# ppwwyyxx/OpenPano

Hardware: NVIDIA H100
Metric: Mpixels/sec SIFT+match+blend (higher is better)
Workload: dtype f32

## Files before the change

openpano_b200/csrc/blur_tile.cuh:

```cuda
#pragma once
#include "common.cuh"

#define BT_W 64
#define BT_H 32
#define BT_THREADS 256

struct BlurTile { int om; int tx, ty; };

__device__ __forceinline__ BlurTile find_blur_tile(const int2* __restrict__ span, int n_om, int cta) {
  int lo = 0, hi = n_om - 1;
  while (lo < hi) {
    const int mid = (lo + hi + 1) >> 1;
    if (span[mid].x <= cta) lo = mid; else hi = mid - 1;
  }
  const int local = cta - span[lo].x, tx_n = span[lo].y;
  BlurTile t;
  t.om = lo; t.ty = local / tx_n; t.tx = local - t.ty * tx_n;
  return t;
}

__device__ __forceinline__ float2 fmul2(float2 a, float t) { return make_float2(__fmul_rn(a.x, t), __fmul_rn(a.y, t)); }

#define BLUR_COLBUF_FLOATS(C) (16 * ((((BT_W + 2 * (C) + 2) / 2) * 2) | 1) * 2)

template <int C>
__device__ __forceinline__ void blur_level(const float* __restrict__ grey, float* __restrict__ colbuf,
                                           float* __restrict__ outT, const float* __restrict__ taps_g,
                                           int R, int RX, int GW, int tid) {
  constexpr int KW = 2 * C + 1;
  float tap[KW];
#pragma unroll
  for (int k = 0; k < KW; ++k) tap[k] = taps_g[k];
  const int start = (RX - C) & ~1, off = (RX - C) - start;
  const int npair = (BT_W + 2 * C + off + 1) >> 1;
  const int csp = (2 * npair) | 1;
  float2* colbuf2 = reinterpret_cast<float2*>(colbuf);
  for (int item = tid; item < (BT_H / 8) * npair; item += BT_THREADS) {
    const int strip = item / npair, pr = item - strip * npair;
    const float2* col = reinterpret_cast<const float2*>(grey + (strip * 8 + R - C) * GW + start) + pr;
    const int gw2 = GW >> 1;
    float2 win[8 + 2 * C];
#pragma unroll
    for (int j = 0; j < 8 + 2 * C; ++j) win[j] = col[j * gw2];
#pragma unroll
    for (int r = 0; r < 8; r += 2) {
      float a0x = 0.f, a0y = 0.f, a1x = 0.f, a1y = 0.f;
#pragma unroll
      for (int k = 0; k < KW; ++k) {
        const float2 p0 = fmul2(win[r + k], tap[k]);
        const float2 p1 = fmul2(win[r + 1 + k], tap[k]);
        a0x += p0.x; a0y += p0.y; a1x += p1.x; a1y += p1.y;
      }
      float2* dst = colbuf2 + (strip * 4 + (r >> 1)) * csp + 2 * pr;
      dst[0] = make_float2(a0x, a1x);
      dst[1] = make_float2(a0y, a1y);
    }
  }
  __syncthreads();
  if (tid < 128) {
    const int lane = tid & 31, p = lane & 15, xs = ((tid >> 5) * 2 + (lane >> 4)) * 8;
    const float2* row = colbuf2 + p * csp + off + xs;
    float2 win[8 + 2 * C];
#pragma unroll
    for (int j = 0; j < 8 + 2 * C; ++j) win[j] = row[j];
#pragma unroll
    for (int c = 0; c < 8; ++c) {
      float ax = 0.f, ay = 0.f;
#pragma unroll
      for (int k = 0; k < KW; ++k) {
        const float2 pp = fmul2(win[c + k], tap[k]);
        ax += pp.x; ay += pp.y;
      }
      outT[(2 * p) * (BT_W + 1) + xs + c] = ax;
      outT[(2 * p + 1) * (BT_W + 1) + xs + c] = ay;
    }
  }
  __syncthreads();
}

__device__ __forceinline__ uint32_t sm_u32(const void* p) { return (uint32_t)__cvta_generic_to_shared(p); }
__device__ __forceinline__ void sbar_init(uint32_t bar, uint32_t count) {
  asm volatile("mbarrier.init.shared::cta.b64 [%0], %1;" ::"r"(bar), "r"(count));
}
__device__ __forceinline__ void sbar_expect_tx(uint32_t bar, uint32_t bytes) {
  asm volatile("mbarrier.arrive.expect_tx.shared::cta.b64 _, [%0], %1;" ::"r"(bar), "r"(bytes) : "memory");
}
__device__ __forceinline__ void sbar_wait(uint32_t bar, uint32_t parity) {
  uint32_t done = 0;
  for (uint32_t spin = 0; spin < (1u << 28); ++spin) {
    asm volatile(
        "{\n\t.reg .pred P1;\n\t"
        "mbarrier.try_wait.parity.shared::cta.b64 P1, [%1], %2;\n\t"
        "selp.b32 %0, 1, 0, P1;\n\t}"
        : "=r"(done) : "r"(bar), "r"(parity) : "memory");
    if (done) return;
  }
  __trap();
}
__device__ __forceinline__ void tma_load_2d(uint32_t dst, const TmaDesc* map, int cx, int cy, uint32_t bar) {
  asm volatile("fence.proxy.tensormap::generic.acquire.gpu [%0], 128;" ::"l"(map) : "memory");
  asm volatile(
      "cp.async.bulk.tensor.2d.shared::cluster.global.tile.mbarrier::complete_tx::bytes [%0], [%1, {%2, %3}], [%4];"
      ::"r"(dst), "l"(map), "r"(cx), "r"(cy), "r"(bar) : "memory");
}
```

openpano_b200/csrc/sift.cu:

```cuda
#include "sift.cuh"
#include "desc_interval.h"
#include <math.h>
#include <string.h>
#include <algorithm>
#include <map>
#include <mutex>
#include <cuda.h>

__device__ __forceinline__ void bilinear_coef(int d, float inv, int src_n, int* s, float* frac) {
  float r = ((float)d + 0.5f) * inv - 0.5f;
  int si = (int)floorf(r);
  r -= (float)si;
  if (si < 0) { si = 0; r = 0.f; }
  else if (si + 1 >= src_n) { si = src_n - 2; r = 1.f; }
  *s = si; *frac = r;
}

__device__ __forceinline__ int first_tap_at_least(int t, float inv, int src_n, int dst_n) {
  auto tap = [&](int d) { int s; float f; bilinear_coef(d, inv, src_n, &s, &f); return s; };
  int d = (int)fminf(fmaxf(((float)t + 0.5f) / inv - 0.5f, 0.f), (float)dst_n);
  while (d > 0 && tap(d - 1) >= t) --d;
  while (d < dst_n && tap(d) < t) ++d;
  return d;
}
// ... 52 lines not shown
    if (lc <= last_c) {
      int sy; float ry;
      bilinear_coef(C0 + lc, im.ify, im.in_w, &sy, &ry);
      for (int lr = threadIdx.x / PG_TW; lr <= last_r; lr += PG_ROWS_PER_PASS) stage(lr, lc, sy, ry);
    }
    const int hr = (int)threadIdx.x - (PG_THREADS - PG_TW);
    if (hr >= 0 && hr <= last_r && PG_TW <= last_c) {
      int sy; float ry;
      bilinear_coef(C0 + PG_TW, im.ify, im.in_w, &sy, &ry);
      stage(hr, PG_TW, sy, ry);
    }
  }
  if (n_oct == 1) return;
  __syncthreads();
  for (int o = 1; o < n_oct; ++o) {
    const OctMeta& om = octs[blockIdx.z * n_oct + o];
    const float ifx = om.ifx, ify = om.ify;
    const int d_r0 = first_tap_at_least(R0, ifx, im.h0, om.h), d_r1 = first_tap_at_least(R0 + PG_TH, ifx, im.h0, om.h);
    const int d_c0 = first_tap_at_least(C0, ify, im.w0, om.w), d_c1 = first_tap_at_least(C0 + PG_TW, ify, im.w0, om.w);
    const int nc = d_c1 - d_c0;
    if (nc == 0) continue;
    float* g = arena + om.gauss_off;
    const int pitch = om.pitch;
    const int step_r = PG_THREADS / nc, step_c = PG_THREADS - step_r * nc;
    int dr = d_r0 + (int)threadIdx.x / nc, dc = d_c0 + (int)threadIdx.x % nc;
    for (; dr < d_r1; dr += step_r, dc += step_c) {
      if (dc >= d_c1) { dc -= nc; ++dr; if (dr >= d_r1) break; }
      int sx, sy; float rx, ry;
      bilinear_coef(dr, ifx, im.h0, &sx, &rx);
      bilinear_coef(dc, ify, im.w0, &sy, &ry);
      const float irx = 1.0f - rx, iry = 1.0f - ry;
      const float* p0 = tile + (sx - R0) * SW + (sy - C0);
      const float* p1 = p0 + SW;
      float v[3];
#pragma unroll
      for (int ch = 0; ch < 3; ++ch)
        v[ch] = rx * (p1[ch * SP + 1] * ry + p1[ch * SP] * iry) + irx * (p0[ch * SP + 1] * ry + p0[ch * SP] * iry);
      g[(size_t)dr * pitch + dc] = (v[0] + v[1] + v[2]) / 3.f;
    }
  }
}

struct ExtremaParams {
  int nscale;
  float pre_color_thres, diff_thres;
  int cap;
  int* cand_count;
  uint32_t* cand_keys;
  int seam_cap;
  int* seam_count;
  uint32_t* seam_keys;
};

__device__ __forceinline__ uint32_t make_key(int oct, int scale, int y, int x) {
  return ((uint32_t)oct << 29) | ((uint32_t)scale << 26) | ((uint32_t)y << 13) | (uint32_t)x;
}

template <class DoG>
__device__ __forceinline__ bool is_extremum(float center, float pre_color_thres, float diff_thres, const DoG& dog) {
  if (center < pre_color_thres) return false;
  const float cmp1 = center - diff_thres, cmp2 = center + diff_thres;
  bool mx = true, mn = true;
#pragma unroll
  for (int ds = -1; ds <= 1; ++ds) {
#pragma unroll
    for (int di = -1; di <= 1; ++di)
#pragma unroll
      for (int dj = -1; dj <= 1; ++dj) {
        if (ds == 0 && di == 0 && dj == 0) continue;
        const float v = dog(ds, di, dj);
        if (v >= cmp1) mx = false;
        if (v <= cmp2) mn = false;
      }
    if (!mx && !mn) return false;
  }
  return true;
}

__device__ __forceinline__ void append_candidate(const ExtremaParams& ep, int img, uint32_t key) {
  const int slot = atomicAdd(&ep.cand_count[img], 1);
  if (slot < ep.cap) ep.cand_keys[(size_t)img * ep.cap + slot] = key;
}

#include "blur_tile.cuh"

__global__ void __launch_bounds__(BT_THREADS)
k_blur_dog(const OctMeta* __restrict__ octs, const int2* __restrict__ span, int n_om,
           float* __restrict__ arena, const __grid_constant__ GaussTable gt) {
  extern __shared__ float smem[];
  const BlurTile tl = find_blur_tile(span, n_om, blockIdx.x);
  const OctMeta om = octs[tl.om];
  const int R = gt.rmax;
  const int GW = BT_W + 2 * R;
  const int GH = BT_H + 2 * R;
  float* grey = smem;
  float* colbuf = smem + GH * GW;
  const int x0 = tl.tx * BT_W, y0 = tl.ty * BT_H;
  const float* g0 = arena + om.gauss_off;
  const int tid = threadIdx.x;

  for (int i = tid; i < GH * GW; i += BT_THREADS) {
    int yy = i / GW, xx = i - yy * GW;
    int gy = min(max(y0 + yy - R, 0), om.h - 1);
    int gx = min(max(x0 + xx - R, 0), om.w - 1);
    grey[i] = __ldg(g0 + (size_t)gy * om.pitch + gx);
  }
  __syncthreads();

  const int tx = tid & (BT_W - 1), ty = tid / BT_W;
  for (int s = 0; s < gt.nlev; ++s) {
    const int c = gt.center[s];
    const float* taps = gt.taps[s];
    const int cw = BT_W + 2 * c;
    for (int i = tid; i < BT_H * cw; i += BT_THREADS) {
      int y = i / cw, xx = i - y * cw;
      const float* col = grey + (y + R - c) * GW + (xx + R - c);
      float tmp = 0.f;
      for (int k = 0; k <= 2 * c; ++k) tmp += col[k * GW] * taps[k];
      colbuf[y * GW + xx] = tmp;
    }
    __syncthreads();
    float* lvl = arena + om.gauss_off + (size_t)(s + 1) * om.plane;
#pragma unroll
    for (int i = 0; i < BT_H / 4; ++i) {
      int y = ty + 4 * i;
      const float* row = colbuf + y * GW + tx;
      float tmp = 0.f;
      for (int k = 0; k <= 2 * c; ++k) tmp += row[k] * taps[k];
      int gx = x0 + tx, gy = y0 + y;
      if (gx < om.w && gy < om.h) lvl[(size_t)gy * om.pitch + gx] = tmp;
    }
    __syncthreads();
  }
}

#define EX_RING_FLOATS (3 * BT_H * BT_W)
__global__ void __launch_bounds__(BT_THREADS, 3)
k_blur_extrema(const OctMeta* __restrict__ octs, const int2* __restrict__ span, int n_om, int n_tiles,
               const TmaDesc* __restrict__ maps, float* __restrict__ arena, const __grid_constant__ GaussTable gt,
               const ExtremaParams ep) {
  extern __shared__ __align__(128) float smem[];
  __shared__ __align__(8) uint64_t s_bar[2];
  __shared__ BlurTile s_tile[2];
  const int R = gt.rmax;
  const int RX = (R + 3) & ~3;
  const int GW = BT_W + 2 * RX, GH = BT_H + 2 * R;
  const int GSZ = (GH * GW + 31) & ~31;
  float* grey0 = smem;
  float* colbuf = smem + 2 * GSZ;
  float* outT = colbuf + BLUR_COLBUF_FLOATS(6);
  float* ring = outT + BT_H * (BT_W + 1);
  const int tid = threadIdx.x;
  const uint32_t tile_bytes = (uint32_t)(GH * GW * sizeof(float));
  int t = blockIdx.x;
  if (tid == 0) {
    sbar_init(sm_u32(&s_bar[0]), 1);
    sbar_init(sm_u32(&s_bar[1]), 1);
    asm volatile("fence.mbarrier_init.release.cluster;" ::: "memory");
    if (t < n_tiles) {
      const BlurTile tl = find_blur_tile(span, n_om, t);
      s_tile[0] = tl;
      sbar_expect_tx(sm_u32(&s_bar[0]), tile_bytes);
      tma_load_2d(sm_u32(grey0), maps + tl.om, tl.tx * BT_W - RX, tl.ty * BT_H - R, sm_u32(&s_bar[0]));
    }
  }
  __syncthreads();
  for (int it = 0; t < n_tiles; t += gridDim.x, ++it) {
    const int b = it & 1;
    float* grey = grey0 + b * GSZ;
    const BlurTile tl = s_tile[b];
    const OctMeta om = octs[tl.om];
    const int x0 = tl.tx * BT_W, y0 = tl.ty * BT_H;
    if (tid == 0 && t + (int)gridDim.x < n_tiles) {
      const BlurTile nx = find_blur_tile(span, n_om, t + gridDim.x);
      s_tile[b ^ 1] = nx;
      asm volatile("fence.proxy.async.shared::cta;" ::: "memory");
      sbar_expect_tx(sm_u32(&s_bar[b ^ 1]), tile_bytes);
      tma_load_2d(sm_u32(grey0 + (b ^ 1) * GSZ), maps + nx.om, nx.tx * BT_W - RX, nx.ty * BT_H - R, sm_u32(&s_bar[b ^ 1]));
    }
    sbar_wait(sm_u32(&s_bar[b]), (uint32_t)(it >> 1) & 1u);
    if (x0 - RX < 0 || y0 - R < 0 || x0 + BT_W + RX > om.w || y0 + BT_H + R > om.h) {
      for (int i = tid; i < GH * GW; i += BT_THREADS) {
        const int yy = i / GW, xx = i - yy * GW;
        const int gy = y0 + yy - R, gx = x0 + xx - RX;
        const int cy = min(max(gy, 0), om.h - 1), cx = min(max(gx, 0), om.w - 1);
        if (cy != gy || cx != gx) grey[i] = grey[(cy - y0 + R) * GW + (cx - x0 + RX)];
      }
      __syncthreads();
    }
    const int tx = tid & (BT_W - 1), ty = tid / BT_W;
    const int gx = x0 + tx;
    const bool col_in = gx >= 1 && gx <= om.w - 2;
    const bool col_seam = tx == 0 || tx == BT_W - 1;
    float prev[BT_H / 4];
#pragma unroll
    for (int i = 0; i < BT_H / 4; ++i) prev[i] = grey[(ty + 4 * i + R) * GW + tx + RX];
    for (int s = 0; s < gt.nlev; ++s) {
      if (gt.center[s] == 3) blur_level<3>(grey, colbuf, outT, gt.taps[s], R, RX, GW, tid);
      else blur_level<6>(grey, colbuf, outT, gt.taps[s], R, RX, GW, tid);
      float* lvl = arena + om.gauss_off + (size_t)(s + 1) * om.plane;
      float* dog = ring + (s % 3) * (BT_H * BT_W);
#pragma unroll
      for (int i = 0; i < BT_H / 4; ++i) {
        const int y = ty + 4 * i, gy = y0 + y;
        const float v = outT[y * (BT_W + 1) + tx];
        if (gx < om.w && gy < om.h) lvl[(size_t)gy * om.pitch + gx] = v;
        dog[y * BT_W + tx] = fabsf(prev[i] - v);
        prev[i] = v;
      }
      if (s >= 2) {
        __syncthreads();
        const int j = s - 1;
        const float* d0 = ring + ((s - 2) % 3) * (BT_H * BT_W);
        const float* d1 = ring + ((s - 1) % 3) * (BT_H * BT_W);
        const float* d2 = dog;
#pragma unroll 1
        for (int i = 0; i < BT_H / 4; ++i) {
          const int y = ty + 4 * i, gy = y0 + y;
          if (!col_in || gy < 1 || gy > om.h - 2) continue;
          const int o = y * BT_W + tx;
          const float center = d1[o];
          if (center < ep.pre_color_thres) continue;
          if (col_seam || y == 0 || y == BT_H - 1) {
            const int slot = atomicAdd(&ep.seam_count[om.img], 1);
            if (slot < ep.seam_cap) ep.seam_keys[(size_t)om.img * ep.seam_cap + slot] = make_key(om.oct, j, gy, gx);
            continue;
          }
          auto at = [&](int ds, int di, int dj) {
            const float* d = ds < 0 ? d0 : ds == 0 ? d1 : d2;
            return d[o + di * BT_W + dj];
          };
          if (is_extremum(center, ep.pre_color_thres, ep.diff_thres, at))
            append_candidate(ep, om.img, make_key(om.oct, j, gy, gx));
        }
      }
    }
    __syncthreads();
  }
}

__device__ __forceinline__ void test_from_levels(const ExtremaParams& ep, const OctMeta& om, const float* arena,
                                                 int j, int gy, int gx, float center) {
  const float* c = arena + om.gauss_off + (size_t)gy * om.pitch + gx;
  auto at = [&](int ds, int di, int dj) {
    const float* q = c + (ptrdiff_t)(j + ds) * om.plane + (ptrdiff_t)di * om.pitch + dj;
    return fabsf(__ldg(q) - __ldg(q + om.plane));
  };
  if (is_extremum(center, ep.pre_color_thres, ep.diff_thres, at))
    append_candidate(ep, om.img, make_key(om.oct, j, gy, gx));
}

__global__ void __launch_bounds__(256)
k_extrema_seams(const OctMeta* __restrict__ octs, int n_oct, const float* __restrict__ arena, const ExtremaParams ep) {
  const int img = blockIdx.y;
  const int n = min(ep.seam_count[img], ep.seam_cap);
  for (int i = blockIdx.x * blockDim.x + threadIdx.x; i < n; i += gridDim.x * blockDim.x) {
    const uint32_t key = ep.seam_keys[(size_t)img * ep.seam_cap + i];
    const int oct = key >> 29, j = (key >> 26) & 7, gy = (key >> 13) & 8191, gx = key & 8191;
    const OctMeta om = octs[img * n_oct + oct];
    const float* c = arena + om.gauss_off + (size_t)gy * om.pitch + gx;
    test_from_levels(ep, om, arena, j, gy, gx, fabsf(__ldg(c + (size_t)j * om.plane) - __ldg(c + (size_t)(j + 1) * om.plane)));
  }
}

#define EXS_THREADS 192

__global__ void __launch_bounds__(EXS_THREADS, 6)
k_extrema_scan(const OctMeta* __restrict__ octs, const int2* __restrict__ span, int n_om,
               const float* __restrict__ arena, const ExtremaParams ep) {
  const BlurTile tl = find_blur_tile(span, n_om, blockIdx.x);
  const OctMeta om = octs[tl.om];
  const int x0 = tl.tx * BT_W, y0 = tl.ty * BT_H;
  for (int p = threadIdx.x; p < BT_W * BT_H; p += EXS_THREADS) {
    const int gx = x0 + (p & (BT_W - 1)), gy = y0 + p / BT_W;
    if (gx < 1 || gx > om.w - 2 || gy < 1 || gy > om.h - 2) continue;
    const float* c = arena + om.gauss_off + (size_t)gy * om.pitch + gx;
    float lv[SIFT_MAX_LEVELS];
#pragma unroll
    for (int l = 1; l < SIFT_MAX_LEVELS; ++l) lv[l] = l <= ep.nscale - 2 ? __ldg(c + (size_t)l * om.plane) : 0.f;
#pragma unroll
    for (int j = 1; j < SIFT_MAX_LEVELS - 1; ++j) {
      if (j >= ep.nscale - 2) break;
      test_from_levels(ep, om, arena, j, gy, gx, fabsf(lv[j] - lv[j + 1]));
    }
  }
}

__global__ void __launch_bounds__(256)
k_rank_sort(const int* __restrict__ cand_count, const uint32_t* __restrict__ keys,
            uint32_t* __restrict__ sorted, int cap) {
  __shared__ uint32_t sk[1024];
  const int img = blockIdx.y;
  const int n = min(cand_count[img], cap);
  const uint32_t* k = keys + (size_t)img * cap;
  for (int c0 = blockIdx.x * 256; c0 < n; c0 += gridDim.x * 256) {
    const int i = c0 + threadIdx.x;
    uint32_t mine = i < n ? k[i] : 0xffffffffu;
    int rank = 0;
    for (int base = 0; base < n; base += 1024) {
      int m = min(1024, n - base);
      __syncthreads();
      for (int t = threadIdx.x; t < m; t += blockDim.x) sk[t] = k[base + t];
      __syncthreads();
      for (int t = 0; t < m; ++t) rank += sk[t] < mine;
    }
    if (i < n) sorted[(size_t)img * cap + rank] = mine;
  }
}

__device__ bool lu3_inverse(const double* a_in, double* inv) {
  double a[9];
  int rowperm[3] = {0, 1, 2}, colperm[3] = {0, 1, 2};
  int nonzero = 3, rank = 0;
  double maxpivot = 0.0;
  for (int i = 0; i < 9; ++i) a[i] = a_in[i];
  for (int k = 0; k < 3; ++k) {
    int br = k, bc = k;
    double big = -1.0;
    for (int i = k; i < 3; ++i)
      for (int j = k; j < 3; ++j) {
// ... 676 lines not shown
  std::vector<int> key = sift_plan_key(n, channels, w, h, p, cap);
  SiftPlan* plan = nullptr;
  if (!keep) {
    plan = ctx->sift_plan;
    ctx->sift_plan = nullptr;
    ctx->sift_plan_bytes = 0;
    if (plan && plan->key != key) { sift_plan_free(ctx, plan); plan = nullptr; }
  }
  const bool fresh = plan == nullptr;

#define SIFT_FAIL(...) do { sift_plan_free(ctx, plan); return ctx_fail(ctx, __VA_ARGS__); } while (0)
#define SIFT_TRY(call) do { int _rc = (call); if (_rc != 0) { sift_plan_free(ctx, plan); return _rc; } } while (0)
#define SIFT_CUDA(call) do { cudaError_t _e = (call); if (_e != cudaSuccess) { int _rc = ctx_cuda(ctx, _e, #call); sift_plan_free(ctx, plan); return _rc; } } while (0)

  std::vector<int2> tilespan;
  if (fresh) {
    plan = new SiftPlan;
    plan->key = std::move(key);
    SiftWork* wk = plan->wk = new SiftWork;
    wk->n_img = n; wk->n_oct = n_oct; wk->n_scale = n_scale; wk->cap = cap;
    wk->h_img.resize(n);
    wk->h_oct.resize((size_t)n * n_oct);
    size_t off = 0;
    int max_w0 = 0, max_h0 = 0;
    int n_tiles = 0;
    size_t seam_cap = 0;
    tilespan.resize((size_t)n * n_oct);
    for (int i = 0; i < n; ++i) {
      if (w[i] < 2 || h[i] < 2) SIFT_FAIL(PANO_ERR_INVALID, "sift: image too small");
      if (channels && (channels[i] != 1 && channels[i] != 3))
        SIFT_FAIL(PANO_ERR_INVALID, "sift: image %d has %d channels (1 or 3)", i, channels[i]);
      ImgMeta& im = wk->h_img[i];
      im.channels = channels ? channels[i] : 3;
      im.in_w = w[i]; im.in_h = h[i];
      float ratio = p->sift_working_size * 2.0f / (w[i] + h[i]);
      im.h0 = (int)(h[i] * ratio); im.w0 = (int)(w[i] * ratio);
      if (im.w0 < 8 || im.h0 < 8 || im.w0 > 8191 || im.h0 > 8191) SIFT_FAIL(PANO_ERR_INVALID, "sift: working size out of range");
      float fx = (float)im.h0 / h[i], fy = (float)im.w0 / w[i];
      im.ifx = 1.f / fx; im.ify = 1.f / fy;
      im.work_off = (long long)off;
      if (keep) off += align_up((size_t)im.w0 * im.h0 * 3, 32);
      max_w0 = std::max(max_w0, im.w0); max_h0 = std::max(max_h0, im.h0);
      size_t img_tiles = 0;
      for (int o = 0; o < n_oct; ++o) {
        OctMeta& om = wk->h_oct[(size_t)i * n_oct + o];
        om.img = i; om.oct = o;
        if (o == 0) { om.w = im.w0; om.h = im.h0; om.ifx = om.ify = 1.f; }
        else {
          float factor = (float)pow((double)p->scale_factor, (double)-o);
          om.w = (int)ceilf(im.w0 * factor); om.h = (int)ceilf(im.h0 * factor);
          if (om.w <= 5 || om.h <= 5) SIFT_FAIL(PANO_ERR_INVALID, "sift: octave too small");
          float ofx = (float)om.h / im.h0, ofy = (float)om.w / im.w0;
          om.ifx = 1.f / ofx; om.ify = 1.f / ofy;
        }
        om.pitch = (int)align_up((size_t)om.w, 32);
        om.plane = (long long)om.pitch * om.h;
        om.gauss_off = (long long)off; off += (size_t)om.plane * n_scale;
        tilespan[(size_t)i * n_oct + o] = make_int2(n_tiles, ceil_div(om.w, BT_W));
        n_tiles += ceil_div(om.w, BT_W) * ceil_div(om.h, BT_H);
        img_tiles += (size_t)ceil_div(om.w, BT_W) * ceil_div(om.h, BT_H);
      }
      seam_cap = std::max(seam_cap, img_tiles * (2 * BT_W + 2 * (BT_H - 2)) * (size_t)(n_scale - 3));
    }
    wk->arena_floats = off;
    wk->n_tiles = n_tiles;
    plan->seam_cap = seam_cap;
    plan->max_w0 = max_w0; plan->max_h0 = max_h0;

    GaussTable& gt = plan->gt;
    memset(&gt, 0, sizeof(gt));
    gt.nlev = n_scale - 1;
    {
      float sigma = p->gauss_sigma;
      for (int s = 0; s < gt.nlev; ++s) {
        int kw = host_gauss_kernel(sigma, p->gauss_window_factor, gt.taps[s], SIFT_MAX_TAPS);
        if (kw < 0) SIFT_FAIL(PANO_ERR_INVALID, "sift: gaussian window %d too wide", -kw);
        gt.center[s] = kw / 2;
        gt.rmax = std::max(gt.rmax, kw / 2);
        sigma *= p->scale_factor;
      }
    }
    plan->fast = true;
    for (int s = 0; s < gt.nlev; ++s) plan->fast = plan->fast && (gt.center[s] == 3 || gt.center[s] == 6);
    const int R = gt.rmax;
    if (((size_t)(BT_H + 2 * R) * (BT_W + 2 * R) + (size_t)BT_H * (BT_W + 2 * R)) * sizeof(float) > 200 * 1024)
      SIFT_FAIL(PANO_ERR_INVALID, "sift: blur halo too large");

    const size_t nlist = (size_t)n * cap;
    SIFT_TRY(plan_alloc(ctx, plan, (void**)&wk->arena, off * sizeof(float)));
    SIFT_TRY(plan_alloc(ctx, plan, (void**)&wk->d_img, n * sizeof(ImgMeta)));
    SIFT_TRY(plan_alloc(ctx, plan, (void**)&wk->d_oct, wk->h_oct.size() * sizeof(OctMeta)));
    SIFT_TRY(plan_alloc(ctx, plan, (void**)&wk->d_maps, (size_t)n * n_oct * sizeof(TmaDesc)));
    SIFT_TRY(plan_alloc(ctx, plan, (void**)&wk->d_tilespan, tilespan.size() * sizeof(int2)));
    SIFT_TRY(plan_alloc(ctx, plan, (void**)&wk->cand_count, (2 * n + 2) * sizeof(int)));
    SIFT_TRY(plan_alloc(ctx, plan, (void**)&wk->seam_keys, (size_t)n * seam_cap * sizeof(uint32_t)));
    SIFT_TRY(plan_alloc(ctx, plan, (void**)&wk->cand_keys, nlist * sizeof(uint32_t)));
    SIFT_TRY(plan_alloc(ctx, plan, (void**)&wk->sorted_keys, nlist * sizeof(uint32_t)));
    SIFT_TRY(plan_alloc(ctx, plan, (void**)&wk->refined, nlist * sizeof(pano_sspoint)));
    SIFT_TRY(plan_alloc(ctx, plan, (void**)&wk->kp_valid, nlist));
    SIFT_TRY(plan_alloc(ctx, plan, (void**)&wk->npeaks, nlist * sizeof(int)));
    SIFT_TRY(plan_alloc(ctx, plan, (void**)&wk->dirs, nlist * SIFT_MAX_PEAKS * sizeof(float)));
    SIFT_TRY(plan_alloc(ctx, plan, (void**)&wk->n_refined, n * sizeof(int)));
    SIFT_TRY(plan_alloc(ctx, plan, (void**)&wk->desc_cand, nlist * sizeof(int)));
    SIFT_TRY(plan_alloc(ctx, plan, (void**)&wk->desc_dir, nlist * sizeof(float)));
  }
  SiftWork* wk = plan->wk;
  const GaussTable& gt = plan->gt;
  const bool fast = plan->fast;
  const size_t seam_cap = plan->seam_cap;
  for (int i = 0; i < n; ++i) {
    if (channels) wk->h_img[i].pix = (const unsigned char*)d_src[i];
    else wk->h_img[i].src = (const float*)d_src[i];
  }

  const size_t nlist = (size_t)n * cap;
  const int n_om = n * n_oct;
  fs->ctx = ctx; fs->n_images = n; fs->cap = cap;
  SIFT_TRY(ctx_alloc(ctx, (void**)&fs->d_desc, nlist * 128 * sizeof(float)));
  SIFT_TRY(ctx_alloc(ctx, (void**)&fs->d_coor, nlist * 4 * sizeof(double)));
  fs->d_real = fs->d_coor + nlist * 2;
  SIFT_TRY(ctx_alloc(ctx, (void**)&fs->d_count, n * sizeof(int)));
  fs->base.resize(n);
  for (int i = 0; i < n; ++i) fs->base[i] = (long long)i * cap;

  {
    void* dsts[4] = {wk->d_img, wk->cand_count, wk->d_oct, wk->d_tilespan};
    const void* srcs[4] = {wk->h_img.data(), nullptr, wk->h_oct.data(), tilespan.data()};
    size_t sizes[4] = {n * sizeof(ImgMeta), (2 * n + 2) * sizeof(int), wk->h_oct.size() * sizeof(OctMeta),
                       tilespan.size() * sizeof(int2)};
    SIFT_TRY(ctx_put_many(ctx, fresh ? 4 : 2, dsts, srcs, sizes));
  }
  if (fresh && fast) {
    std::vector<TmaDesc> maps(n_om);
    const int R = gt.rmax;
    for (int k = 0; k < n_om; ++k) {
      const OctMeta& om = wk->h_oct[k];
      unsigned long long dims[2] = {(unsigned long long)om.w, (unsigned long long)om.h};
      unsigned long long strides[1] = {(unsigned long long)om.pitch * sizeof(float)};
      unsigned box[2] = {(unsigned)(BT_W + 2 * ((R + 3) & ~3)), (unsigned)(BT_H + 2 * R)};
      SIFT_TRY(ctx_tma_encode(ctx, &maps[k], wk->arena + om.gauss_off, 2, dims, strides, box));
    }
    SIFT_TRY(ctx_put(ctx, wk->d_maps, maps.data(), maps.size() * sizeof(TmaDesc)));
  }

#define SIFT_LAUNCH(name, kernel, grid, block, smem, ...)                                   \
  do {                                                                                      \
    ctx->launches++;                                                                        \
    if (ctx->profiling) ctx_prof_begin(ctx, name);                                          \
    kernel<<<(grid), (block), (smem), ctx->stream>>>(__VA_ARGS__);                          \
    if (ctx->profiling) ctx_prof_end(ctx);                                                  \
    SIFT_CUDA(cudaGetLastError());                                                          \
  } while (0)

  {
    dim3 g(ceil_div(plan->max_w0, PG_TW), ceil_div(plan->max_h0, PG_TH), n);
    float* work = keep ? wk->arena : nullptr;
    if (channels)
      SIFT_LAUNCH("k_pyramid_grey_rgb8", k_pyramid_grey<SrcRgb8>, g, PG_THREADS, 0, wk->d_img, wk->d_oct, n_oct, wk->arena, work);
    else
      SIFT_LAUNCH("k_pyramid_grey", k_pyramid_grey<SrcF32>, g, PG_THREADS, 0, wk->d_img, wk->d_oct, n_oct, wk->arena, work);
  }
  {
    const ExtremaParams ep{n_scale, p->pre_color_thres, p->judge_extrema_diff_thres, cap, wk->cand_count, wk->cand_keys,
                           (int)seam_cap, wk->cand_count + n + 2, wk->seam_keys};
    const int R = gt.rmax;
    size_t smem = ((size_t)(BT_H + 2 * R) * (BT_W + 2 * R) + (size_t)BT_H * (BT_W + 2 * R)) * sizeof(float);
    if (fast) {
      const int GW = BT_W + 2 * ((R + 3) & ~3), GH = BT_H + 2 * R;
      const size_t gsz = ((size_t)GH * GW + 31) & ~(size_t)31;
      size_t smf = (2 * gsz + (size_t)BLUR_COLBUF_FLOATS(6) + (size_t)BT_H * (BT_W + 1) + EX_RING_FLOATS) * sizeof(float);
      SIFT_CUDA(sift_smem_limit(ctx, (const void*)k_blur_extrema, smf));
      const int grid = std::min(wk->n_tiles, ctx->num_sms * 3);
      SIFT_LAUNCH("k_blur_extrema", k_blur_extrema, grid, BT_THREADS, smf, wk->d_oct, wk->d_tilespan, n_om, wk->n_tiles,
                  wk->d_maps, wk->arena, gt, ep);
      SIFT_LAUNCH("k_extrema_seams", k_extrema_seams, dim3(8, n), 256, 0, wk->d_oct, n_oct, wk->arena, ep);
    } else {
      if (smem > 48 * 1024)
        SIFT_CUDA(sift_smem_limit(ctx, (const void*)k_blur_dog, smem));
      SIFT_LAUNCH("k_blur_dog_generic", k_blur_dog, wk->n_tiles, BT_THREADS, smem, wk->d_oct, wk->d_tilespan, n_om, wk->arena, gt);
      SIFT_LAUNCH("k_extrema_scan", k_extrema_scan, wk->n_tiles, EXS_THREADS, 0, wk->d_oct, wk->d_tilespan, n_om,
                  wk->arena, ep);
    }
  }
  {
    dim3 g(8, n);
    SIFT_LAUNCH("k_rank_sort", k_rank_sort, g, 256, 0, wk->cand_count, wk->cand_keys, wk->sorted_keys, cap);
    RefineParams rp{n_scale, p->calc_offset_depth, p->offset_thres, p->contrast_thres, p->edge_ratio,
                    p->gauss_sigma, p->scale_factor};
    dim3 g4(16, n);
    SIFT_LAUNCH("k_refine", k_refine, g4, 128, 0, wk->d_oct, wk->arena, n_oct, wk->cand_count, wk->sorted_keys, rp, cap,
                wk->refined, wk->kp_valid);
    SIFT_LAUNCH("k_orientation", k_orientation, ctx->num_sms * 8, ORI_WARPS * 32, 0, wk->d_oct, wk->arena, n_oct, n, cap,
                wk->cand_count, wk->refined, wk->kp_valid, p->ori_radius, p->ori_hist_smooth_count, wk->npeaks, wk->dirs,
                wk->cand_count + n + 1);
    SIFT_LAUNCH("k_expand_scan", k_expand_scan, n, SCAN_THREADS, 0, wk->cand_count, wk->kp_valid, wk->npeaks,
                wk->dirs, cap, fs->d_count, wk->n_refined, wk->desc_cand, wk->desc_dir);
    DescParams dp{p->desc_hist_scale_factor, p->desc_int_factor};
    const size_t dsm = sizeof(DescQuadSmem) * DESC_WARPS;
    SIFT_CUDA(sift_smem_limit(ctx, (const void*)k_descriptor, dsm));
    const int grid = ctx->num_sms * DESC_MIN_CTAS;
    SIFT_LAUNCH("k_descriptor", k_descriptor, grid, DESC_THREADS, dsm, wk->d_oct, wk->d_img, wk->arena, n_oct, n, cap,
                wk->refined, fs->d_count, wk->desc_cand, wk->desc_dir, dp, fs->d_desc, fs->d_coor, wk->cand_count + n);
  }
  wk->n_desc = fs->d_count;

  if (!fs->h_count_pinned) {
    fs->h_count_pinned = (int*)ctx_small_pinned_get(ctx, (size_t)2 * n * sizeof(int) + 16, &fs->h_count_cap);
    if (!fs->h_count_pinned) SIFT_FAIL(PANO_ERR_CUDA, "pinned allocation failed");
  }
  {
    void* dsts[2] = {fs->h_count_pinned, fs->h_count_pinned + n};
    const void* srcs[2] = {fs->d_count, wk->cand_count};
    size_t sizes[2] = {n * sizeof(int), n * sizeof(int)};
    SIFT_TRY(ctx_store_many(ctx, 2, dsts, srcs, sizes));
  }
  SIFT_CUDA(ctx_signal(ctx, &fs->counts_token));
  fs->counts_pending = true;
  fs->counts_on_host = false;

  if (keep) {
    *keep = wk;
    plan->wk = nullptr;
    delete plan;
  } else if (ctx->cache_limit && plan->bytes <= ctx->cache_limit) {
    ctx->sift_plan = plan;
    ctx->sift_plan_bytes = plan->bytes;
    if (ctx->cached_bytes + plan->bytes > ctx->cache_limit) ctx_cache_release(ctx, ctx->cache_limit - plan->bytes);
  } else {
    sift_plan_free(ctx, plan);
  }
  return PANO_OK;
#undef SIFT_FAIL
#undef SIFT_TRY
#undef SIFT_CUDA
#undef SIFT_LAUNCH
}


int featureset_sync_counts(pano_featureset* fs) {
  SlowCall sc("featureset_sync_counts");
  if (fs->error) return fs->error;
  if (fs->counts_on_host) return PANO_OK;
  pano_ctx* ctx = fs->ctx;
  while (fs->counts_pending) {
    cudaError_t e = ctx_wait_signal(ctx, fs->counts_token);
    if (e != cudaSuccess) return fs->error = ctx_cuda(ctx, e, "feature count read-back");
    fs->counts_pending = false;
    const int n = fs->n_images;
    int worst = 0;
    for (int i = 0; i < n; ++i) worst = std::max(worst, std::max(fs->h_count_pinned[i], fs->h_count_pinned[n + i]));
    if (worst <= fs->cap) {
      fs->h_count.assign(fs->h_count_pinned, fs->h_count_pinned + n);
      break;
    }
    int cap = fs->cap;
// ... 17 lines not shown
```

openpano_b200/csrc/sift.cuh:

```cuda
#pragma once
#include "common.cuh"
#include "match_tc.cuh"

#define SIFT_MAX_OCT 8
#define SIFT_MAX_LEVELS 8
#define SIFT_MAX_TAPS 32
#define SIFT_CAP_DEFAULT 8192
#define SIFT_CAP_MAX (1 << 20)
#define SIFT_MAX_PEAKS 18

struct ImgMeta {
  union {
    const float* src;
    const unsigned char* pix;
  };
  int in_w, in_h;
  int w0, h0;
  float ifx, ify;
  long long work_off;
  int channels;
};

struct OctMeta {
  int img, oct;
  int w, h;
  int pitch;
  float ifx, ify;
  long long gauss_off;
  long long plane;
};

struct GaussTable {
  int nlev;
  int rmax;
  int center[SIFT_MAX_LEVELS];
  float taps[SIFT_MAX_LEVELS][SIFT_MAX_TAPS];
};

struct SiftWork {
  int n_img = 0, n_oct = 0, n_scale = 0;
  std::vector<ImgMeta> h_img;
  std::vector<OctMeta> h_oct;
  float* arena = nullptr;
  size_t arena_floats = 0;
  ImgMeta* d_img = nullptr;
  OctMeta* d_oct = nullptr;
  int2* d_tilespan = nullptr;
  TmaDesc* d_maps = nullptr;
  int n_tiles = 0;
  int cap = SIFT_CAP_DEFAULT;
  int* cand_count = nullptr;
  uint32_t* cand_keys = nullptr;
  uint32_t* seam_keys = nullptr;
  uint32_t* sorted_keys = nullptr;
  pano_sspoint* refined = nullptr;
  unsigned char* kp_valid = nullptr;
  int* npeaks = nullptr;
  float* dirs = nullptr;
  int* n_desc = nullptr;
  int* n_refined = nullptr;
  int* desc_cand = nullptr;
  float* desc_dir = nullptr;
};

struct SiftPlan {
  std::vector<int> key;
  SiftWork* wk = nullptr;
  size_t bytes = 0;
  GaussTable gt;
  bool fast = true;
  size_t seam_cap = 0;
  int max_w0 = 0, max_h0 = 0;
};

struct pano_featureset {
  pano_ctx* ctx = nullptr;
  int n_images = 0;
  float* d_desc = nullptr;
  double* d_coor = nullptr;
  double* d_real = nullptr;
  int* d_count = nullptr;
  std::vector<long long> base;
  std::vector<int> h_count;
  bool counts_on_host = false;
  cudaEvent_t counts_ready = nullptr;
  unsigned counts_token = 0;
  bool counts_pending = false;
  int* h_count_pinned = nullptr;
  size_t h_count_cap = 0;
  TcOperands tc;
  bool tc_ready = false;
  int error = 0;
  int cap = 0;
  std::vector<const void*> src;
  std::vector<int> src_channels;
  std::vector<int> src_w, src_h;
  pano_params src_params;
  void* owned_block = nullptr;
};

int sift_run_batch(pano_ctx* ctx, int n, const void* const* d_src, const int* channels, const int* w, const int* h,
                   const pano_params* p, pano_featureset* fs, SiftWork** keep, int cap);
void sift_work_free(pano_ctx* ctx, SiftWork* wk);
void sift_plan_free(pano_ctx* ctx, SiftPlan* plan);
int featureset_sync_counts(pano_featureset* fs);
```

Before: 11270.

## Group blur levels per pass, drop TMA double buffer, warp-aggregate extrema appends

Restructures the fused blur+extrema kernel to blur up to three Gaussian levels of the same tap width per pass, sharing one sync pair and writing the horizontal pass straight into a five-slot DoG ring instead of an outT staging buffer. The TMA double buffer becomes a single buffer whose next tile is prefetched only after the last group's blur. Gaussian outputs are stored as float4, and candidate and seam keys are appended through warp-level prefix sums with one atomic per warp. Occupancy drops from 3 to 2 CTAs per SM, and tile-load overlap now covers only the final extrema scan.

```diff
diff --git a/openpano_b200/csrc/blur_tile.cuh b/openpano_b200/csrc/blur_tile.cuh
--- a/openpano_b200/csrc/blur_tile.cuh
+++ b/openpano_b200/csrc/blur_tile.cuh
@@ -24,6 +24,31 @@
 #define BLUR_COLBUF_FLOATS(C) (16 * ((((BT_W + 2 * (C) + 2) / 2) * 2) | 1) * 2)
 
 template <int C>
+__device__ __forceinline__ void blur_col_item(const float* __restrict__ grey, float2* __restrict__ colbuf2,
+                                              const float (&tap)[2 * C + 1], int strip, int pr, int R, int GW,
+                                              int start, int csp) {
+  constexpr int KW = 2 * C + 1;
+  const float2* col = reinterpret_cast<const float2*>(grey + (strip * 8 + R - C) * GW + start) + pr;
+  const int gw2 = GW >> 1;
+  float2 win[8 + 2 * C];
+#pragma unroll
+  for (int j = 0; j < 8 + 2 * C; ++j) win[j] = col[j * gw2];
+#pragma unroll
+  for (int r = 0; r < 8; r += 2) {
+    float a0x = 0.f, a0y = 0.f, a1x = 0.f, a1y = 0.f;
+#pragma unroll
+    for (int k = 0; k < KW; ++k) {
+      const float2 p0 = fmul2(win[r + k], tap[k]);
+      const float2 p1 = fmul2(win[r + 1 + k], tap[k]);
+      a0x += p0.x; a0y += p0.y; a1x += p1.x; a1y += p1.y;
+    }
+    float2* dst = colbuf2 + (strip * 4 + (r >> 1)) * csp + 2 * pr;
+    dst[0] = make_float2(a0x, a1x);
+    dst[1] = make_float2(a0y, a1y);
+  }
+}
+
+template <int C>
 __device__ __forceinline__ void blur_level(const float* __restrict__ grey, float* __restrict__ colbuf,
                                            float* __restrict__ outT, const float* __restrict__ taps_g,
                                            int R, int RX, int GW, int tid) {
@@ -37,24 +62,7 @@
   float2* colbuf2 = reinterpret_cast<float2*>(colbuf);
   for (int item = tid; item < (BT_H / 8) * npair; item += BT_THREADS) {
     const int strip = item / npair, pr = item - strip * npair;
-    const float2* col = reinterpret_cast<const float2*>(grey + (strip * 8 + R - C) * GW + start) + pr;
-    const int gw2 = GW >> 1;
-    float2 win[8 + 2 * C];
-#pragma unroll
-    for (int j = 0; j < 8 + 2 * C; ++j) win[j] = col[j * gw2];
-#pragma unroll
-    for (int r = 0; r < 8; r += 2) {
-      float a0x = 0.f, a0y = 0.f, a1x = 0.f, a1y = 0.f;
-#pragma unroll
-      for (int k = 0; k < KW; ++k) {
-        const float2 p0 = fmul2(win[r + k], tap[k]);
-        const float2 p1 = fmul2(win[r + 1 + k], tap[k]);
-        a0x += p0.x; a0y += p0.y; a1x += p1.x; a1y += p1.y;
-      }
-      float2* dst = colbuf2 + (strip * 4 + (r >> 1)) * csp + 2 * pr;
-      dst[0] = make_float2(a0x, a1x);
-      dst[1] = make_float2(a0y, a1y);
-    }
+    blur_col_item<C>(grey, colbuf2, tap, strip, pr, R, GW, start, csp);
   }
   __syncthreads();
   if (tid < 128) {
diff --git a/openpano_b200/csrc/sift.cu b/openpano_b200/csrc/sift.cu
--- a/openpano_b200/csrc/sift.cu
+++ b/openpano_b200/csrc/sift.cu
@@ -158,6 +158,23 @@
   if (slot < ep.cap) ep.cand_keys[(size_t)img * ep.cap + slot] = key;
 }
 
+template <class Key>
+__device__ __forceinline__ void append_keys_warp(int* count, uint32_t* keys, int cap, unsigned bits, const Key& key) {
+  if (__ballot_sync(0xffffffffu, bits != 0) == 0) return;
+  const int lane = threadIdx.x & 31, n = __popc(bits);
+  int incl = n;
+#pragma unroll
+  for (int d = 1; d < 32; d <<= 1) {
+    const int v = __shfl_up_sync(0xffffffffu, incl, d);
+    if (lane >= d) incl += v;
+  }
+  int base = 0;
+  if (lane == 31) base = atomicAdd(count, incl);
+  int slot = __shfl_sync(0xffffffffu, base, 31) + incl - n;
+  for (; bits; bits &= bits - 1, ++slot)
+    if (slot < cap) keys[slot] = key(__ffs(bits) - 1);
+}
+
 #include "blur_tile.cuh"
 
 __global__ void __launch_bounds__(BT_THREADS)
@@ -210,51 +227,90 @@
   }
 }
 
-#define EX_RING_FLOATS (3 * BT_H * BT_W)
-__global__ void __launch_bounds__(BT_THREADS, 3)
+#define EX_GROUP 3
+#define EX_SL (BT_W + 4)
+#define EX_SLOT (BT_H * EX_SL)
+#define EX_SLOTS (EX_GROUP + 2)
+#define EX_CTAS_PER_SM 2
+static_assert(EX_SLOT % 32 == 0 && BLUR_COLBUF_FLOATS(6) % 32 == 0, "slots start on 128-byte lines");
+
+template <int C, class Emit>
+__device__ __forceinline__ void blur_group(const float* __restrict__ grey, float* __restrict__ colbuf,
+                                           const GaussTable& gt, int a, int g, int R, int RX, int GW, int tid,
+                                           int p, int xs, const Emit& emit) {
+  constexpr int KW = 2 * C + 1;
+  constexpr int CB = BLUR_COLBUF_FLOATS(6);
+  const int start = (RX - C) & ~1, off = (RX - C) - start;
+  const int npair = (BT_W + 2 * C + off + 1) >> 1;
+  const int csp = (2 * npair) | 1;
+  const int nitem = (BT_H / 8) * npair;
+  for (int item = tid; item < g * nitem; item += BT_THREADS) {
+    const int l = item / nitem, rest = item - l * nitem;
+    const int strip = rest / npair, pr = rest - strip * npair;
+    float tap[KW];
+#pragma unroll
+    for (int k = 0; k < KW; ++k) tap[k] = gt.taps[a + l][k];
+    blur_col_item<C>(grey, reinterpret_cast<float2*>(colbuf + l * CB), tap, strip, pr, R, GW, start, csp);
+  }
+  __syncthreads();
+  for (int l = 0; l < g; ++l) {
+    float tap[KW];
+#pragma unroll
+    for (int k = 0; k < KW; ++k) tap[k] = gt.taps[a + l][k];
+    const float2* row = reinterpret_cast<const float2*>(colbuf + l * CB) + p * csp + off + xs;
+    float2 win[4 + 2 * C];
+#pragma unroll
+    for (int j = 0; j < 4 + 2 * C; ++j) win[j] = row[j];
+    float ax[4], ay[4];
+#pragma unroll
+    for (int c = 0; c < 4; ++c) {
+      ax[c] = 0.f; ay[c] = 0.f;
+#pragma unroll
+      for (int k = 0; k < KW; ++k) {
+        const float2 pp = fmul2(win[c + k], tap[k]);
+        ax[c] += pp.x; ay[c] += pp.y;
+      }
+    }
+    emit(l, ax, ay);
+  }
+  __syncthreads();
+}
+
+__global__ void __launch_bounds__(BT_THREADS, EX_CTAS_PER_SM)
 k_blur_extrema(const OctMeta* __restrict__ octs, const int2* __restrict__ span, int n_om, int n_tiles,
                const TmaDesc* __restrict__ maps, float* __restrict__ arena, const __grid_constant__ GaussTable gt,
                const ExtremaParams ep) {
   extern __shared__ __align__(128) float smem[];
-  __shared__ __align__(8) uint64_t s_bar[2];
-  __shared__ BlurTile s_tile[2];
+  __shared__ __align__(8) uint64_t s_bar;
+  __shared__ BlurTile s_tile;
   const int R = gt.rmax;
   const int RX = (R + 3) & ~3;
   const int GW = BT_W + 2 * RX, GH = BT_H + 2 * R;
   const int GSZ = (GH * GW + 31) & ~31;
-  float* grey0 = smem;
-  float* colbuf = smem + 2 * GSZ;
-  float* outT = colbuf + BLUR_COLBUF_FLOATS(6);
-  float* ring = outT + BT_H * (BT_W + 1);
+  float* grey = smem;
+  float* colbuf = smem + GSZ;
+  float* slots = colbuf + EX_GROUP * BLUR_COLBUF_FLOATS(6);
   const int tid = threadIdx.x;
   const uint32_t tile_bytes = (uint32_t)(GH * GW * sizeof(float));
+  auto stage = [&](int t) {
+    const BlurTile tl = find_blur_tile(span, n_om, t);
+    s_tile = tl;
+    asm volatile("fence.proxy.async.shared::cta;" ::: "memory");
+    sbar_expect_tx(sm_u32(&s_bar), tile_bytes);
+    tma_load_2d(sm_u32(grey), maps + tl.om, tl.tx * BT_W - RX, tl.ty * BT_H - R, sm_u32(&s_bar));
+  };
   int t = blockIdx.x;
   if (tid == 0) {
-    sbar_init(sm_u32(&s_bar[0]), 1);
-    sbar_init(sm_u32(&s_bar[1]), 1);
+    sbar_init(sm_u32(&s_bar), 1);
     asm volatile("fence.mbarrier_init.release.cluster;" ::: "memory");
-    if (t < n_tiles) {
-      const BlurTile tl = find_blur_tile(span, n_om, t);
-      s_tile[0] = tl;
-      sbar_expect_tx(sm_u32(&s_bar[0]), tile_bytes);
-      tma_load_2d(sm_u32(grey0), maps + tl.om, tl.tx * BT_W - RX, tl.ty * BT_H - R, sm_u32(&s_bar[0]));
-    }
+    if (t < n_tiles) stage(t);
   }
   __syncthreads();
   for (int it = 0; t < n_tiles; t += gridDim.x, ++it) {
-    const int b = it & 1;
-    float* grey = grey0 + b * GSZ;
-    const BlurTile tl = s_tile[b];
+    sbar_wait(sm_u32(&s_bar), (uint32_t)it & 1u);
+    const BlurTile tl = s_tile;
     const OctMeta om = octs[tl.om];
     const int x0 = tl.tx * BT_W, y0 = tl.ty * BT_H;
-    if (tid == 0 && t + (int)gridDim.x < n_tiles) {
-      const BlurTile nx = find_blur_tile(span, n_om, t + gridDim.x);
-      s_tile[b ^ 1] = nx;
-      asm volatile("fence.proxy.async.shared::cta;" ::: "memory");
-      sbar_expect_tx(sm_u32(&s_bar[b ^ 1]), tile_bytes);
-      tma_load_2d(sm_u32(grey0 + (b ^ 1) * GSZ), maps + nx.om, nx.tx * BT_W - RX, nx.ty * BT_H - R, sm_u32(&s_bar[b ^ 1]));
-    }
-    sbar_wait(sm_u32(&s_bar[b]), (uint32_t)(it >> 1) & 1u);
     if (x0 - RX < 0 || y0 - R < 0 || x0 + BT_W + RX > om.w || y0 + BT_H + R > om.h) {
       for (int i = tid; i < GH * GW; i += BT_THREADS) {
         const int yy = i / GW, xx = i - yy * GW;
@@ -268,50 +324,66 @@
     const int gx = x0 + tx;
     const bool col_in = gx >= 1 && gx <= om.w - 2;
     const bool col_seam = tx == 0 || tx == BT_W - 1;
-    float prev[BT_H / 4];
-#pragma unroll
-    for (int i = 0; i < BT_H / 4; ++i) prev[i] = grey[(ty + 4 * i + R) * GW + tx + RX];
-    for (int s = 0; s < gt.nlev; ++s) {
-      if (gt.center[s] == 3) blur_level<3>(grey, colbuf, outT, gt.taps[s], R, RX, GW, tid);
-      else blur_level<6>(grey, colbuf, outT, gt.taps[s], R, RX, GW, tid);
-      float* lvl = arena + om.gauss_off + (size_t)(s + 1) * om.plane;
-      float* dog = ring + (s % 3) * (BT_H * BT_W);
-#pragma unroll
-      for (int i = 0; i < BT_H / 4; ++i) {
-        const int y = ty + 4 * i, gy = y0 + y;
-        const float v = outT[y * (BT_W + 1) + tx];
-        if (gx < om.w && gy < om.h) lvl[(size_t)gy * om.pitch + gx] = v;
-        dog[y * BT_W + tx] = fabsf(prev[i] - v);
-        prev[i] = v;
-      }
-      if (s >= 2) {
-        __syncthreads();
-        const int j = s - 1;
-        const float* d0 = ring + ((s - 2) % 3) * (BT_H * BT_W);
-        const float* d1 = ring + ((s - 1) % 3) * (BT_H * BT_W);
-        const float* d2 = dog;
-#pragma unroll 1
+    const int lane = tid & 31, p = lane & 15, xs = ((tid >> 5) * 2 + (lane >> 4)) * 4;
+    float prev[2][4];
+#pragma unroll
+    for (int r = 0; r < 2; ++r)
+#pragma unroll
+      for (int c = 0; c < 4; ++c) prev[r][c] = grey[(2 * p + r + R) * GW + RX + xs + c];
+    for (int gi = 0; gi < gt.ngroup; ++gi) {
+      const int a = gt.group[gi], g = gt.group[gi + 1] - a;
+      auto emit = [&](int l, const float (&ax)[4], const float (&ay)[4]) {
+        float* lvl = arena + om.gauss_off + (size_t)(a + l + 1) * om.plane;
+        float* dog = slots + ((a + l) % EX_SLOTS) * EX_SLOT + (2 * p) * EX_SL + xs;
+        float v[2][4];
+#pragma unroll
+        for (int c = 0; c < 4; ++c) { v[0][c] = ax[c]; v[1][c] = ay[c]; }
+#pragma unroll
+        for (int r = 0; r < 2; ++r) {
+          *reinterpret_cast<float4*>(dog + r * EX_SL) =
+              make_float4(fabsf(prev[r][0] - v[r][0]), fabsf(prev[r][1] - v[r][1]), fabsf(prev[r][2] - v[r][2]),
+                          fabsf(prev[r][3] - v[r][3]));
+          const int gy = y0 + 2 * p + r, gx0 = x0 + xs;
+          if (gy < om.h) {
+            float* q = lvl + (size_t)gy * om.pitch + gx0;
+            if (gx0 + 3 < om.w) *reinterpret_cast<float4*>(q) = make_float4(v[r][0], v[r][1], v[r][2], v[r][3]);
+            else
+#pragma unroll
+              for (int c = 0; c < 4; ++c)
+                if (gx0 + c < om.w) q[c] = v[r][c];
+          }
+#pragma unroll
+          for (int c = 0; c < 4; ++c) prev[r][c] = v[r][c];
+        }
+      };
+      if (gt.center[a] == 3) blur_group<3>(grey, colbuf, gt, a, g, R, RX, GW, tid, p, xs, emit);
+      else blur_group<6>(grey, colbuf, gt, a, g, R, RX, GW, tid, p, xs, emit);
+      if (gi == gt.ngroup - 1 && tid == 0 && t + (int)gridDim.x < n_tiles) stage(t + gridDim.x);
+      const int j0 = max(a - 1, 1), j1 = a + g - 2;
+      for (int j = j0; j <= j1; ++j) {
+        const float* d0 = slots + ((j - 1) % EX_SLOTS) * EX_SLOT;
+        const float* d1 = slots + (j % EX_SLOTS) * EX_SLOT;
+        const float* d2 = slots + ((j + 1) % EX_SLOTS) * EX_SLOT;
+        unsigned live = 0, seam = 0, cand = 0;
+#pragma unroll
         for (int i = 0; i < BT_H / 4; ++i) {
-          const int y = ty + 4 * i, gy = y0 + y;
-          if (!col_in || gy < 1 || gy > om.h - 2) continue;
-          const int o = y * BT_W + tx;
-          const float center = d1[o];
-          if (center < ep.pre_color_thres) continue;
-          if (col_seam || y == 0 || y == BT_H - 1) {
-            const int slot = atomicAdd(&ep.seam_count[om.img], 1);
-            if (slot < ep.seam_cap) ep.seam_keys[(size_t)om.img * ep.seam_cap + slot] = make_key(om.oct, j, gy, gx);
-            continue;
-          }
+          const int gy = y0 + ty + 4 * i;
+          if (!(d1[(ty + 4 * i) * EX_SL + tx] < ep.pre_color_thres) && col_in && gy >= 1 && gy <= om.h - 2) live |= 1u << i;
+        }
+        for (; live; live &= live - 1) {
+          const int i = __ffs(live) - 1, y = ty + 4 * i, o = y * EX_SL + tx;
+          if (col_seam || y == 0 || y == BT_H - 1) { seam |= 1u << i; continue; }
           auto at = [&](int ds, int di, int dj) {
             const float* d = ds < 0 ? d0 : ds == 0 ? d1 : d2;
-            return d[o + di * BT_W + dj];
+            return d[o + di * EX_SL + dj];
           };
-          if (is_extremum(center, ep.pre_color_thres, ep.diff_thres, at))
-            append_candidate(ep, om.img, make_key(om.oct, j, gy, gx));
+          if (is_extremum(d1[o], ep.pre_color_thres, ep.diff_thres, at)) cand |= 1u << i;
         }
-      }
-    }
-    __syncthreads();
+        auto key = [&](int i) { return make_key(om.oct, j, y0 + ty + 4 * i, gx); };
+        append_keys_warp(ep.seam_count + om.img, ep.seam_keys + (size_t)om.img * ep.seam_cap, ep.seam_cap, seam, key);
+        append_keys_warp(ep.cand_count + om.img, ep.cand_keys + (size_t)om.img * ep.cap, ep.cap, cand, key);
+      }
+    }
   }
 }
 
@@ -1154,6 +1226,14 @@
     }
     plan->fast = true;
     for (int s = 0; s < gt.nlev; ++s) plan->fast = plan->fast && (gt.center[s] == 3 || gt.center[s] == 6);
+    for (int s = 0; s < gt.nlev;) {
+      int e = s;
+      while (e < gt.nlev && gt.center[e] == gt.center[s]) ++e;
+      const int n_run = e - s, parts = (n_run + EX_GROUP - 1) / EX_GROUP;
+      for (int k = 0; k < parts; ++k) gt.group[gt.ngroup++] = s + k * n_run / parts;
+      s = e;
+    }
+    gt.group[gt.ngroup] = gt.nlev;
     const int R = gt.rmax;
     if (((size_t)(BT_H + 2 * R) * (BT_W + 2 * R) + (size_t)BT_H * (BT_W + 2 * R)) * sizeof(float) > 200 * 1024)
       SIFT_FAIL(PANO_ERR_INVALID, "sift: blur halo too large");
@@ -1240,9 +1320,9 @@
     if (fast) {
       const int GW = BT_W + 2 * ((R + 3) & ~3), GH = BT_H + 2 * R;
       const size_t gsz = ((size_t)GH * GW + 31) & ~(size_t)31;
-      size_t smf = (2 * gsz + (size_t)BLUR_COLBUF_FLOATS(6) + (size_t)BT_H * (BT_W + 1) + EX_RING_FLOATS) * sizeof(float);
+      size_t smf = (gsz + (size_t)EX_GROUP * BLUR_COLBUF_FLOATS(6) + (size_t)EX_SLOTS * EX_SLOT) * sizeof(float);
       SIFT_CUDA(sift_smem_limit(ctx, (const void*)k_blur_extrema, smf));
-      const int grid = std::min(wk->n_tiles, ctx->num_sms * 3);
+      const int grid = std::min(wk->n_tiles, ctx->num_sms * EX_CTAS_PER_SM);
       SIFT_LAUNCH("k_blur_extrema", k_blur_extrema, grid, BT_THREADS, smf, wk->d_oct, wk->d_tilespan, n_om, wk->n_tiles,
                   wk->d_maps, wk->arena, gt, ep);
       SIFT_LAUNCH("k_extrema_seams", k_extrema_seams, dim3(8, n), 256, 0, wk->d_oct, n_oct, wk->arena, ep);
diff --git a/openpano_b200/csrc/sift.cuh b/openpano_b200/csrc/sift.cuh
--- a/openpano_b200/csrc/sift.cuh
+++ b/openpano_b200/csrc/sift.cuh
@@ -35,6 +35,8 @@
   int rmax;
   int center[SIFT_MAX_LEVELS];
   float taps[SIFT_MAX_LEVELS][SIFT_MAX_TAPS];
+  int ngroup;
+  int group[SIFT_MAX_LEVELS + 1];
 };
 
 struct SiftWork {
```

Result: no change. 11530 (median of 6 runs) (+2.2%).
